# Shahriar1638/Hybrid-Language-Music-Clustering-VAE

Hardware: AMD Instinct MI355X
Metric: clips/sec mel+VAE train step, 128-mel x 128-frame, bs=256, 1/2/4/8 MI355X (higher is better)
Workload: dtype bf16; 1 GPU; Convolutional_VAE audio-only (BASELINE config[1]): PCM[256,65024] -> HIP mel-dB 128x128 -> z-score -> VAE fwd+bwd+Adam; per_gpu_batch=256, global_batch=256, mel=128x128, params=13304961, parallelism=dp1, world_size=1, launch=single process, pcm_batches=5 distinct batches in rotation (333 MB), execution=eager launches

## Files before the change

### hybrid-language-music-clustering-vae_amd/_lib.py

```python
from __future__ import annotations

import ctypes as C
import os

import numpy as np
import torch

_HERE = os.path.dirname(os.path.abspath(__file__))
LIB_PATH = os.environ.get("HLMC_LIB") or os.path.join(_HERE, "libhlmc.so")

c_int, c_i64, c_f32, c_f64, c_vp, c_char_p = C.c_int, C.c_int64, C.c_float, C.c_double, C.c_void_p, C.c_char_p
P_vp = C.POINTER(c_vp)
P_i64 = C.POINTER(c_i64)

HLMC_F32, HLMC_BF16 = 0, 1
NET_HYBRID, NET_CVAE, NET_SIMPLE = 0, 1, 2

_SIGS = {
    "hlmc_version": (c_int, []),
    "hlmc_last_error": (c_char_p, []),
    "hlmc_device_status": (c_int, [c_int]),
    "hlmc_test_bn_fused": (c_int, [c_i64, c_int]),
    "hlmc_mel_plan_create": (c_int, [c_int, c_int, c_int, c_int, c_f64, c_f64, P_vp]),
    "hlmc_mel_plan_destroy": (c_int, [c_vp]),
    "hlmc_mel_filterbank": (c_int, [c_vp, c_vp]),
    "hlmc_mel_frames": (c_i64, [c_vp, c_i64]),
    "hlmc_mel_workspace": (c_i64, [c_vp, c_i64, c_i64]),
    "hlmc_melspectrogram": (c_int, [c_vp, c_vp, c_vp, c_i64, c_i64, c_vp, c_vp]),
    "hlmc_mel_db": (c_int, [c_vp, c_vp, c_vp, c_i64, c_i64, c_i64, c_f32, c_f32, c_vp, c_vp]),
    "hlmc_mel_db_zscore": (c_int, [c_vp, c_vp, c_vp, c_i64, c_i64, c_i64, c_f32, c_f32, c_vp, c_vp, c_int, c_vp,
                                   c_vp]),
    "hlmc_power_to_db": (c_int, [c_vp, c_vp, c_i64, c_i64, c_int, c_f32, c_f32, c_f32, c_vp, c_vp]),
    "hlmc_mfcc": (c_int, [c_vp, c_vp, c_vp, c_i64, c_i64, c_int, c_vp, c_vp]),
    "hlmc_spectral_shape": (c_int, [c_vp, c_vp, c_vp, c_i64, c_i64, c_f64, c_vp]),
    "hlmc_zcr_rms": (c_int, [c_vp, c_vp, c_vp, c_i64, c_i64, c_vp, c_vp]),
    "hlmc_chroma_workspace": (c_i64, [c_vp, c_i64, c_i64]),
    "hlmc_chroma_stft": (c_int, [c_vp, c_vp, c_vp, c_i64, c_i64, c_vp, c_vp, c_vp]),
    "hlmc_row_mean_std": (c_int, [c_vp, c_vp, c_i64, c_i64, c_vp, c_vp]),
    "hlmc_colstats_workspace": (c_i64, [c_i64, c_i64]),
    "hlmc_colstats_sum": (c_int, [c_vp, c_vp, c_i64, c_i64, c_vp, c_vp]),
    "hlmc_colstats_centered": (c_int, [c_vp, c_vp, c_i64, c_i64, c_vp, c_vp, c_vp, c_vp]),
    "hlmc_zscore_apply": (c_int, [c_vp, c_vp, c_i64, c_i64, c_vp, c_vp, c_int, c_vp]),
    "hlmc_net_create": (c_int, [c_int, P_i64, c_int, c_int, P_vp]),
    "hlmc_net_destroy": (c_int, [c_vp]),
    "hlmc_net_num_params": (c_int, [c_vp]),
    "hlmc_net_param_info": (c_int, [c_vp, c_int, c_char_p, c_int, C.POINTER(c_int), P_i64]),
    "hlmc_net_num_bn": (c_int, [c_vp]),
    "hlmc_net_state_bytes": (c_i64, [c_vp]),
    "hlmc_net_workspace_bytes": (c_i64, [c_vp, c_i64]),
    "hlmc_net_bind": (c_int, [c_vp, P_vp, P_vp, P_vp, P_vp, c_vp]),
    "hlmc_net_forward": (c_int, [c_vp, c_vp, c_i64, c_int, c_vp, c_vp, c_vp, c_vp, c_vp, c_vp, c_vp, c_vp, c_vp,
                                 c_vp, c_vp]),
    "hlmc_net_encode": (c_int, [c_vp, c_vp, c_i64, c_int, c_vp, c_vp, c_vp, c_vp, c_vp, c_vp]),
    "hlmc_net_decode": (c_int, [c_vp, c_vp, c_i64, c_int, c_vp, c_vp, c_vp, c_vp, c_vp, c_vp]),
    "hlmc_net_backward": (c_int, [c_vp, c_vp, c_i64, c_vp, c_vp, c_vp, c_vp, c_vp]),
    "hlmc_net_adam_step": (c_int, [c_vp, c_vp, P_vp, P_vp, c_f32, c_f32, c_f32, c_f32, c_f32, c_int]),
    "hlmc_net_set_trust_packs": (c_int, [c_vp, c_int]),
    "hlmc_net_adam_step_dev": (c_int, [c_vp, c_vp, P_vp, P_vp, c_vp]),
    "hlmc_adam_coef": (c_int, [c_f32, c_f32, c_f32, c_f32, c_f32, c_int, c_vp]),
    "hlmc_net_set_overlap_adam": (c_int, [c_vp, c_int]),
    "hlmc_net_set_rng": (c_int, [c_vp, C.c_uint64, C.c_uint64]),
    "hlmc_net_get_rng": (c_int, [c_vp, C.POINTER(C.c_uint64), C.POINTER(C.c_uint64)]),
    "hlmc_randn": (c_int, [c_vp, c_vp, c_i64, C.c_uint64, C.c_uint64]),
    "hlmc_net_settle": (c_int, [c_vp, c_vp]),
    "hlmc_net_grad_buckets": (c_int, [c_vp, C.POINTER(c_int), c_int]),
    "hlmc_net_set_bucket_sync": (c_int, [c_vp, c_int]),
    "hlmc_net_bucket_wait": (c_int, [c_vp, c_int, c_vp]),
    "hlmc_probe_arm": (c_int, [c_int, c_int]),
    "hlmc_probe_read": (c_int, [C.POINTER(c_int), C.POINTER(c_f64), C.POINTER(c_f64), C.POINTER(c_f64),
                                C.POINTER(c_f32), c_int]),
    "hlmc_loss_workspace": (c_i64, [c_i64, c_i64, c_i64]),
    "hlmc_loss_sums": (c_int, [c_vp, c_vp, c_vp, c_i64, c_vp, c_vp, c_i64, c_vp, c_vp, c_i64, c_vp, c_vp]),
    "hlmc_loss_backward": (c_int, [c_vp, c_vp, c_vp, c_i64, c_vp, c_vp, c_vp, c_i64, c_vp, c_vp, c_vp, c_i64,
                                   c_vp, c_vp, c_vp]),
    "hlmc_loss_sums_backward": (c_int, [c_vp, c_vp, c_vp, c_i64, c_vp, c_vp, c_vp, c_i64, c_vp, c_vp, c_vp, c_i64,
                                        c_vp, c_vp, c_vp, c_vp, c_vp]),
    "hlmc_adam_scratch_bytes": (c_i64, [c_int]),
    "hlmc_adam_step": (c_int, [c_vp, c_int, P_vp, P_vp, P_vp, P_vp, P_i64, c_f32, c_f32, c_f32, c_f32, c_f32,
                               c_int, c_vp]),
    "hlmc_km_center": (c_int, [c_vp, c_vp, c_i64, c_int, c_vp, c_vp, c_vp]),
    "hlmc_km_sqdist_rows": (c_int, [c_vp, c_vp, c_i64, c_int, P_i64, c_int, c_vp]),
    "hlmc_km_assign": (c_int, [c_vp, c_vp, c_i64, c_int, c_vp, c_int, c_vp, c_vp, c_vp]),
    "hlmc_km_sums": (c_int, [c_vp, c_vp, c_i64, c_int, c_vp, c_int, c_vp, c_vp]),
    "hlmc_km_sums_workspace": (c_i64, [c_i64, c_int]),
    "hlmc_km_sums_part": (c_int, [c_vp, c_vp, c_i64, c_int, c_vp, c_int, c_vp, c_vp, c_vp, c_i64]),
    "hlmc_km_rowdist": (c_int, [c_vp, c_vp, c_i64, c_int, c_vp, c_vp, c_vp]),
    "hlmc_km_inertia": (c_int, [c_vp, c_vp, c_i64, c_int, c_vp, c_vp, c_vp, c_vp]),
    "hlmc_op_bn_bwd_workspace": (c_i64, [c_int]),
    "hlmc_op_bn_bwd": (c_int, [c_vp, c_int, c_vp, c_vp, c_i64, c_int, c_vp, c_vp, c_vp, c_vp, c_vp, c_vp, c_vp, c_vp, c_vp,
                               c_i64]),
    "hlmc_km_assign_batch": (c_int, [c_vp, c_vp, c_i64, c_int, c_vp, c_int, c_int, C.c_uint64, c_vp, c_vp, c_vp]),
    "hlmc_km_sums_batch": (c_int, [c_vp, c_vp, c_i64, c_int, c_vp, c_int, c_int, C.c_uint64, c_vp, c_vp, c_vp, c_i64]),
    "hlmc_km_update_batch": (c_int, [c_vp, c_int, c_int, c_int, C.c_uint64, c_vp, c_vp, c_vp, c_vp, c_vp]),
    "hlmc_km_pp_search": (c_int, [c_vp, c_i64, c_int, c_int, c_vp, c_int, C.POINTER(C.c_int32), C.POINTER(c_f64), c_vp,
                                  c_vp]),
    "hlmc_km_pp_dist": (c_int, [c_vp, c_vp, c_i64, c_int, c_int, c_int, c_vp, c_vp, c_int, C.POINTER(C.c_int32), c_vp]),
    "hlmc_km_inertia_batch": (c_int, [c_vp, c_vp, c_i64, c_int, c_vp, c_int, c_vp, c_int, c_vp, c_vp]),
    "hlmc_silhouette_workspace": (c_i64, [c_i64, c_int]),
    "hlmc_silhouette": (c_int, [c_vp, c_vp, c_i64, c_int, c_vp, c_int, c_vp, c_vp, c_vp, c_i64]),
    "hlmc_cluster_scores_workspace": (c_i64, [c_int, c_int]),
    "hlmc_cluster_scores": (c_int, [c_vp, c_vp, c_i64, c_int, c_vp, c_int, c_vp, c_vp, c_i64]),
    "hlmc_dbscan_workspace": (c_i64, [c_i64, c_int]),
    "hlmc_dbscan_neighbors": (c_int, [c_vp, c_vp, c_i64, c_int, C.POINTER(c_f64), c_int, c_vp, c_vp, c_vp, c_i64]),
    "hlmc_dbscan_labels": (c_int, [c_vp, c_i64, c_int, c_int, c_int, c_vp, c_vp, c_i64, c_vp, c_vp, c_vp]),
    "hlmc_ward_workspace": (c_i64, [c_i64]),
    "hlmc_ward_pdist": (c_int, [c_vp, c_vp, c_i64, c_int, c_vp]),
    "hlmc_ward_chain": (c_int, [c_vp, c_i64, c_vp, c_vp, c_vp, c_vp, c_vp, c_vp, c_i64]),
    "hlmc_pca_workspace": (c_i64, [c_i64, c_int]),
    "hlmc_pca_cov": (c_int, [c_vp, c_vp, c_i64, c_int, c_vp, c_vp, c_vp, c_i64]),
# ... 97 lines not shown
```

### hybrid-language-music-clustering-vae_amd/csrc/capi.cpp

```cpp
#include <algorithm>
#include <cmath>
#include <cstring>
#include <memory>
#include <vector>

#include "engine.hpp"
#include "features.hpp"

namespace hlmc {

static thread_local std::string g_err;
void set_error(const std::string& msg) { g_err = msg; }
const char* get_error() { return g_err.c_str(); }
static int device_status_ok() {
    const unsigned st = ops::dev_status_take(false);
    if (st == 0) return HLMC_OK;
    set_error("device status " + std::to_string(st) +
              (st & kDevBnCountTimeout ? ": a one-launch BatchNorm backward's grid-wide arrival count timed out (grid not "
                                         "co-resident); that launch's dgamma / dbeta / dy are NaN" : "") +
              " -- clear with hlmc_device_status(1)");
    return HLMC_EDEVICE;
}

namespace probe {
// ... 213 lines not shown
    for (int i = 0; i < n.n_bn; ++i) {
        n.RM.push_back(running[2 * i]);
        n.RV.push_back(running[2 * i + 1]);
    }
    n.NBT.assign(nbt, nbt + n.n_bn);
    for (size_t i = 0; i < np; ++i) HLMC_CHECK_ARG(n.P[i] && n.G[i], "NULL parameter / grad pointer");
    n.state = reinterpret_cast<char*>(state);
    n.packs_valid = false;
    return n.bind_state(nullptr);
}
int hlmc_net_forward(hlmc_net* h, void* stream, int64_t batch, int train, const float* in0, const float* in1,
                     const float* in2, const float* eps, const uint8_t* dropout, float* recon, float* recon_text,
                     float* mu, float* logvar, float* z, void* ws) {
    HLMC_CHECK_ARG(h && ws && batch > 0, "bad arguments");
    HLMC_CHECK_ARG(!h->impl->P.empty(), "net is not bound");
    ForwardArgs a{batch, train, in0, in1, in2, eps, dropout, recon, recon_text, mu, logvar, z, ws, false};
    return h->impl->forward(S(stream), a);
}
int hlmc_net_encode(hlmc_net* h, void* stream, int64_t batch, int train, const float* in0, const float* in1,
                    const float* in2, float* mu, float* logvar, void* ws) {
    HLMC_CHECK_ARG(h && ws && batch > 0, "bad arguments");
    HLMC_CHECK_ARG(!h->impl->P.empty(), "net is not bound");
    ForwardArgs a{batch, train, in0, in1, in2, nullptr, nullptr, nullptr, nullptr, mu, logvar, nullptr, ws, true};
    return h->impl->forward(S(stream), a);
}
int hlmc_net_decode(hlmc_net* h, void* stream, int64_t batch, int train, const float* z, const float* cond,
                    const uint8_t* dropout, float* recon, float* recon_text, void* ws) {
    HLMC_CHECK_ARG(h && ws && batch > 0 && z && recon, "bad arguments");
    HLMC_CHECK_ARG(!h->impl->P.empty(), "net is not bound");
    ForwardArgs a{batch, train, z, nullptr, cond, nullptr, dropout, recon, recon_text, nullptr, nullptr, nullptr, ws,
                  false, true};
    return h->impl->forward(S(stream), a);
}
int hlmc_net_backward(hlmc_net* h, void* stream, int64_t batch, const float* d_recon, const float* d_recon_text,
                      const float* d_mu, const float* d_logvar, void* ws) {
    HLMC_CHECK_ARG(h && ws && d_recon && d_mu && d_logvar, "bad arguments");
    HLMC_TRY(device_status_ok());
    BackwardArgs a{batch, d_recon, d_recon_text, d_mu, d_logvar, ws};
    return h->impl->backward(S(stream), a);
}

int hlmc_net_adam_step(hlmc_net* h, void* stream, float* const* exp_avg, float* const* exp_avg_sq, float lr, float b1,
                       float b2, float eps, float wd, int step) {
    HLMC_CHECK_ARG(h && exp_avg && exp_avg_sq && step >= 1, "bad arguments");
    HLMC_CHECK_ARG(!h->impl->P.empty(), "net is not bound");
    return h->impl->adam_step(S(stream), exp_avg, exp_avg_sq, ops::AdamArgs{lr, b1, b2, eps, wd, step});
}
int hlmc_net_adam_step_dev(hlmc_net* h, void* stream, float* const* exp_avg, float* const* exp_avg_sq,
                           const float* coef_dev) {
    HLMC_CHECK_ARG(h && exp_avg && exp_avg_sq && coef_dev, "bad arguments");
    HLMC_CHECK_ARG(!h->impl->P.empty(), "net is not bound");
    return h->impl->adam_step(S(stream), exp_avg, exp_avg_sq, ops::AdamArgs{0.f, 0.f, 0.f, 0.f, 0.f, 1}, coef_dev);
}
int hlmc_adam_coef(float lr, float b1, float b2, float eps, float wd, int step, float* out6) {
    HLMC_CHECK_ARG(out6 && step >= 1, "bad arguments");
    ops::adam_coef_host(ops::AdamArgs{lr, b1, b2, eps, wd, step}, out6);
    return HLMC_OK;
}
int hlmc_net_set_trust_packs(hlmc_net* h, int trust) {
    HLMC_CHECK_ARG(h, "net is NULL");
    h->impl->trust_packs = trust != 0;
    if (!trust) h->impl->packs_valid = false;
    return HLMC_OK;
}
int hlmc_net_settle(hlmc_net* h, void* stream) {
    HLMC_CHECK_ARG(h, "net is NULL");
    return h->impl->settle(S(stream));
}
int hlmc_net_set_rng(hlmc_net* h, uint64_t seed, uint64_t offset) {
    HLMC_CHECK_ARG(h && offset % 4 == 0, "net is NULL / offset not a multiple of 4");
    h->impl->rng_seed = seed;
    h->impl->rng_offset = offset;
    return HLMC_OK;
}
int hlmc_net_get_rng(const hlmc_net* h, uint64_t* seed, uint64_t* offset) {
    HLMC_CHECK_ARG(h && seed && offset, "NULL argument");
    *seed = h->impl->rng_seed;
    *offset = h->impl->rng_offset;
    return HLMC_OK;
}
int hlmc_randn(void* stream, float* out, int64_t n, uint64_t seed, uint64_t offset) {
    return ops::randn(S(stream), out, n, seed, offset);
}
int hlmc_net_set_overlap_adam(hlmc_net* h, int enable) {
    HLMC_CHECK_ARG(h, "net is NULL");
    h->impl->overlap_adam = enable != 0;
    return HLMC_OK;
}
int hlmc_net_grad_buckets(const hlmc_net* h, int* starts, int cap) {
    HLMC_CHECK_ARG(h && starts && cap > 0, "NULL argument");
    const auto& b = h->impl->bucket_starts;
    for (int k = 0; k < (int)b.size() && k < cap; ++k) starts[k] = b[k];
    return (int)b.size();
}
int hlmc_net_set_bucket_sync(hlmc_net* h, int enable) {
    HLMC_CHECK_ARG(h, "net is NULL");
    h->impl->bucket_sync = enable != 0;
    return HLMC_OK;
}
int hlmc_net_bucket_wait(hlmc_net* h, int k, void* stream) {
    HLMC_CHECK_ARG(h, "net is NULL");
    auto& ev = h->impl->bucket_ev;
    HLMC_CHECK_ARG(h->impl->bucket_sync && k >= 0 && k < (int)ev.size() && ev[k],
                   "bucket events not recorded (hlmc_net_set_bucket_sync + hlmc_net_backward first)");
    HLMC_HIP(hipStreamWaitEvent(S(stream), ev[k], 0));
    return HLMC_OK;
// ... 249 lines not shown
```

### hybrid-language-music-clustering-vae_amd/csrc/engine.cpp

```cpp
#include "engine.hpp"

#include <algorithm>
#include <climits>
#include <cstdlib>
#include <functional>

namespace hlmc {
namespace {

constexpr float kBnEps = 1e-5f;
constexpr float kBnMomentum = 0.1f;
constexpr int ENC_CH[7] = {1, 32, 64, 128, 256, 512, 512};
constexpr int DEC_CH[7] = {512, 512, 256, 128, 64, 32, 1};

inline int pad8(int64_t n) { return (int)((n + 7) & ~int64_t(7)); }

struct WgradQueue {
    using Fn = std::function<int(hipStream_t, Ws)>;
    bool on = true;
    Ws ws_main{nullptr, 0};
    Ws ws_own{nullptr, 0};

    WgradQueue() = default;
    WgradQueue(const WgradQueue&) = delete;
// ... 121 lines not shown
            p.ld1 = q.ld1 = pad8(p.d0);
            p.off0 = A.take((size_t)2 * p.d0 * p.ld0 * sizeof(T));
            q.off0 = p.off0 + (size_t)p.d0 * p.ld0 * sizeof(T);
            p.off1 = A.take((size_t)p.d1 * p.ld1 * sizeof(T));
            q.off1 = A.take((size_t)q.d1 * q.ld1 * sizeof(T));
        }
        for (auto& p : packs) {
            if (!p.taps) continue;
            ++njobs;
            if (p.off0 != SIZE_MAX) continue;
            p.ld0 = p.taps == 1 ? pad8(p.d1) : p.d1;
            p.ld1 = p.taps == 1 ? pad8(p.d0) : p.d0;
            p.off0 = A.take((size_t)p.d0 * p.taps * p.ld0 * sizeof(T));
            p.off1 = A.take((size_t)p.d1 * p.taps * p.ld1 * sizeof(T));
        }
        jobs_off = A.take(sizeof(ops::AdamJob) * std::max<size_t>(1, njobs));
        ajobs_off = A.take(sizeof(ops::AdamJob) * std::max<size_t>(1, params.size()));
        state_size = A.used;
    }
    size_t state_bytes() const override { return state_size; }
    ops::AdamJob job_for(size_t i, float* m, float* v) const {
        const Pack& p = packs[i];
        ops::AdamJob j{P[i], G[i], m, v, nullptr, nullptr, params[i].numel(), 0, 0, 0, 0, 0, 0, 0};
        if (p.taps) {
            j.p0 = state + p.off0;
            j.p1 = state + p.off1;
            j.d0 = p.d0; j.d1 = p.d1; j.taps = p.taps; j.ld0 = p.ld0; j.ld1 = p.ld1;
        }
        return j;
    }
    std::vector<ops::AdamJob> pjobs;
    int bind_state(hipStream_t s) override {
        pjobs.clear();
        pack_tiles = 0;
        for (size_t i = 0; i < packs.size(); ++i) {
            if (!packs[i].taps) continue;
            ops::AdamJob j = job_for(i, nullptr, nullptr);
            j.tile0 = pack_tiles;
            pack_tiles += ops::adam_job_tiles(j);
            pjobs.push_back(j);
        }
        if (!pjobs.empty())
            HLMC_HIP(hipMemcpyAsync(state + jobs_off, pjobs.data(), pjobs.size() * sizeof(ops::AdamJob), hipMemcpyHostToDevice, s));
        ajobs_m.clear();
        HLMC_HIP(hipStreamSynchronize(s));
        return HLMC_OK;
    }
    int pack_all(hipStream_t s) {
        if (trust_packs && packs_valid) return HLMC_OK;
        HLMC_TRY(ops::pack<T>(s, reinterpret_cast<const ops::AdamJob*>(state + jobs_off), njobs, pack_tiles));
        packs_valid = true;
        return HLMC_OK;
    }
    int adam_step(hipStream_t s, float* const* m, float* const* v, const ops::AdamArgs& a, const float* coef_dev) override {
        const size_t np = params.size();
        if (ajobs_m.size() != np || !std::equal(ajobs_m.begin(), ajobs_m.end(), m) ||
            !std::equal(ajobs_v.begin(), ajobs_v.end(), v)) {
            ajobs_m.assign(m, m + np);
            ajobs_v.assign(v, v + np);
            ajobs.clear();
            adam_tiles = 0;
            for (size_t i = 0; i < np; ++i) {
                ops::AdamJob j = job_for(i, m[i], v[i]);
                j.tile0 = adam_tiles;
                adam_tiles += ops::adam_job_tiles(j);
                ajobs.push_back(j);
            }
            HLMC_HIP(hipMemcpyAsync(state + ajobs_off, ajobs.data(), ajobs.size() * sizeof(ops::AdamJob),
                                    hipMemcpyHostToDevice, s));
        }
        const auto* jd = reinterpret_cast<const ops::AdamJob*>(state + ajobs_off);
        if (join_pending) {
            const int tsplit = ajobs[this->late_params].tile0;
            HLMC_TRY(wq.wait_prelate(s));
            HLMC_TRY(ops::adam_pack<T>(s, jd, (int)np, adam_tiles, a, coef_dev, tsplit));
            HLMC_TRY(wq.join(s));
            join_pending = false;
            HLMC_TRY(ops::adam_pack<T>(s, jd, (int)np, tsplit, a, coef_dev, 0));
        } else {
            HLMC_TRY(ops::adam_pack<T>(s, jd, (int)np, adam_tiles, a, coef_dev));
        }
        packs_valid = true;
        return HLMC_OK;
    }
    T* P0(int w) const { return reinterpret_cast<T*>(state + packs[w].off0); }
    T* P1(int w) const { return reinterpret_cast<T*>(state + packs[w].off1); }
    int ld0(int w) const { return packs[w].ld0; }
    int ld1(int w) const { return packs[w].ld1; }

    char* ws = nullptr;
    Ws scratch{nullptr, 0};
    size_t scratch_off = 0, scratch2_off = 0, scratch_bytes = 0;
    int64_t planned_B = -1;
    size_t ws_total = 0;

    T* AT(size_t off) const { return reinterpret_cast<T*>(ws + off); }
    float* AF(size_t off) const { return reinterpret_cast<float*>(ws + off); }
    uint8_t* AU8(size_t off) const { return reinterpret_cast<uint8_t*>(ws + off); }

    void need(size_t b) { scratch_bytes = std::max(scratch_bytes, b); }
    size_t xf_total = 0, xb_total = 0, xf_base = 0, xb_base = 0;
    bool bwd_acc_clean = false;
    int zero_acc_fwd(hipStream_t s) {
        if (xf_total + xb_total) HLMC_HIP(hipMemsetAsync(ws + xf_base, 0, xf_total + xb_total, s));
        bwd_acc_clean = true;
        return HLMC_OK;
    }
    int zero_acc_bwd(hipStream_t s) {
        if (!bwd_acc_clean && xb_total) HLMC_HIP(hipMemsetAsync(ws + xb_base, 0, xb_total, s));
        bwd_acc_clean = false;
        return HLMC_OK;
    }

    virtual void plan(Arena& A, int64_t B) = 0;
    size_t ws_bytes(int64_t B) override {
        if (B != planned_B) {
            Arena A;
            scratch_bytes = 0;
            xf_total = xb_total = 0;
            plan(A, B);
            scratch_off = A.take(scratch_bytes + 256);
            scratch2_off = A.take(scratch_bytes + 256);
            xf_base = A.take(xf_total);
            xb_base = A.take(xb_total);
            ws_total = A.used;
            planned_B = B;
        }
        return ws_total;
    }
    void set_ws(void* w) {
        ws = reinterpret_cast<char*>(w);
        scratch = Ws{reinterpret_cast<float*>(ws + scratch_off), scratch_bytes + 256};
        wq.ws_main = scratch;
        wq.ws_own = Ws{reinterpret_cast<float*>(ws + scratch2_off), scratch_bytes + 256};
    }

    WgradQueue wq;
    bool join_pending = false;
    ~NetT() override {
        for (auto e : this->bucket_ev) (void)hipEventDestroy(e);
    }
    static constexpr int side_batch() { return 2; }
    static constexpr int dense_batch() { return 2; }
    bool tail_overlap() const { return wq.on && this->overlap_adam && !this->bucket_sync && this->late_params > 0; }
    int prelate(hipStream_t s) { return tail_overlap() ? wq.record_prelate(s) : (int)HLMC_OK; }
    int settle(hipStream_t s) override {
        if (!join_pending) return HLMC_OK;
        join_pending = false;
        return wq.join(s);
    }
    int finish_backward(hipStream_t s) {
        if (tail_overlap()) {
            join_pending = true;
            return HLMC_OK;
        }
        return wq.join(s);
    }
    int mark(hipStream_t s, int k) {
        if (!this->bucket_sync) return HLMC_OK;
        HLMC_CHECK_ARG(k >= 0 && k < (int)this->bucket_ev.size(), "bucket index");
        if (wq.on && k + 1 < (int)this->bucket_ev.size()) return wq.record_bucket(s, this->bucket_ev[k]);
        HLMC_HIP(hipEventRecord(this->bucket_ev[k], s));
        return HLMC_OK;
    }

    int begin_forward(hipStream_t s, const ForwardArgs& a) {
        HLMC_CHECK_ARG(a.B >= 2 || !a.train, "BatchNorm in train mode needs batch >= 2");
        ws_bytes((int)a.B);
        set_ws(a.ws);
        HLMC_TRY(settle(s));
        HLMC_TRY(pack_all(s));
        if (a.train) HLMC_TRY(zero_acc_fwd(s));
        this->last_full_forward = !a.encode_only && !a.decode_only;
        return HLMC_OK;
    }
    int begin_backward(hipStream_t s, const BackwardArgs& a) {
        HLMC_CHECK_ARG((int)a.B == planned_B, "backward batch differs from the last forward");
        HLMC_CHECK_ARG(this->last_full_forward, "backward needs a full hlmc_net_forward (not encode / decode)");
        set_ws(a.ws);
        HLMC_TRY(wq.init());
        if (this->bucket_sync && this->bucket_ev.size() != this->bucket_starts.size()) {
            for (auto e : this->bucket_ev) (void)hipEventDestroy(e);
            this->bucket_ev.assign(this->bucket_starts.size(), nullptr);
            for (auto& e : this->bucket_ev) HLMC_HIP(hipEventCreateWithFlags(&e, hipEventDisableTiming));
        }
        HLMC_TRY(settle(s));
        return zero_acc_bwd(s);
    }

    int reparam(hipStream_t s, const float* eps_in, const float* mu, const float* lv, float* eps_keep, int B, int L,
                T* z, int ldz, float* mu_out, float* lv_out) {
        if (eps_in) return ops::reparam_fwd<T>(s, mu, lv, eps_in, B, L, z, ldz, mu_out, lv_out, eps_keep);
        return ops::reparam_rng<T>(s, mu, lv, this->rng_seed, take_rng(B, L), B, L, eps_keep, z, ldz, mu_out, lv_out);
    }
    uint64_t take_rng(int B, int L) {
        const uint64_t off = this->rng_offset;
        this->rng_offset += ((uint64_t)B * L + 3) & ~uint64_t(3);
        return off;
    }
    int latent_out(hipStream_t s, const ForwardArgs& a, const float* mu, const float* lv, int64_t nl) {
        const ops::CopySeg cs[2] = {{a.mu, mu, nl}, {a.logvar, lv, nl}};
        return ops::copy_segments(s, cs, 2);
    }
    int heads_fwd(hipStream_t s, const ForwardArgs& a, const T* x, int ldx, int B, int L, int mu_w, int mu_b, int lv_b,
                  float* mu, float* lv, float* eps_keep, T* z, int ldz) {
        const int K = (int)params[mu_w].shape[1];
        int S = 0;
        HLMC_TRY(ops::linear_partials<T>(s, x, ldx, B, K, P0(mu_w), ld0(mu_w), 2 * L, scratch, &S));
        if (a.encode_only)
            return ops::heads_reparam<T>(s, scratch.p, S, B, L, P[mu_b], P[lv_b], mu, lv, a.mu, a.logvar, nullptr, 0, 0,
                                         nullptr, nullptr, 0);
// ... 934 lines not shown
```

### hybrid-language-music-clustering-vae_amd/csrc/engine.hpp

```cpp
#pragma once
#include <memory>
#include <string>
#include <vector>

#include "ops.hpp"

namespace hlmc {

struct ParamInfo {
    std::string name;
    std::vector<int64_t> shape;
    int64_t numel() const {
        int64_t n = 1;
        for (auto d : shape) n *= d;
        return n;
    }
};

struct Arena {
    size_t used = 0;
    size_t take(size_t bytes) {
        size_t o = used;
        used += (bytes + 255) & ~size_t(255);
        return o;
// ... 1 lines not shown
};

struct ForwardArgs {
    int64_t B;
    int train;
    const float* in0;
    const float* in1;
    const float* in2;
    const float* eps;
    const uint8_t* dropout;
    float* recon;
    float* recon_text;
    float* mu;
    float* logvar;
    float* z;
    void* ws;
    bool encode_only;
    bool decode_only = false;
};

struct BackwardArgs {
    int64_t B;
    const float* d_recon;
    const float* d_recon_text;
    const float* d_mu;
    const float* d_logvar;
    void* ws;
};

class NetBase {
  public:
    virtual ~NetBase() = default;
    int kind = 0, dtype = 0;
    std::vector<ParamInfo> params;
    int n_bn = 0;

    std::vector<float*> P, G, RM, RV;
    std::vector<int64_t*> NBT;
    char* state = nullptr;

    int add_param(const std::string& name, std::vector<int64_t> shape) {
        params.push_back({name, std::move(shape)});
        return (int)params.size() - 1;
    }
    int add_bn() { return n_bn++; }

    virtual size_t state_bytes() const = 0;
    virtual size_t ws_bytes(int64_t B) = 0;
    virtual int bind_state(hipStream_t s) = 0;
    virtual int forward(hipStream_t s, const ForwardArgs& a) = 0;
    virtual int backward(hipStream_t s, const BackwardArgs& a) = 0;
    virtual int adam_step(hipStream_t s, float* const* m, float* const* v, const ops::AdamArgs& a,
                          const float* coef_dev = nullptr) = 0;
    bool trust_packs = false;
    bool packs_valid = false;

    std::vector<int> bucket_starts{0};
    std::vector<hipEvent_t> bucket_ev;
    bool bucket_sync = false;

    int late_params = 0;
    bool overlap_adam = false;
    bool last_full_forward = false;
    uint64_t rng_seed = 0, rng_offset = 0;
    virtual int settle(hipStream_t s) = 0;
};

int make_net(int kind, const int64_t* cfg, int ncfg, int dtype, std::unique_ptr<NetBase>* out);

}
```

### hybrid-language-music-clustering-vae_amd/train.py

```python
from __future__ import annotations

import os

import torch

from . import _lib as L
from .models import ConditionalVAE, HybridVAE, VAE


class Trainer:
    def __init__(self, model, lr=1e-4, betas=(0.9, 0.999), eps=1e-8, weight_decay=0.0, beta=None, text_weight=None,
                 process_group=None, distributed=False, grad_dtype=torch.float32, broadcast_buffers=True):
        self.model = model
        self.distributed = distributed or process_group is not None
        self.process_group = process_group
        self.broadcast_buffers = bool(broadcast_buffers) and self.distributed
        self.bn_flat = model._flatten_bn_buffers() if self.broadcast_buffers else None
        self.kind = "simple" if isinstance(model, VAE) else ("cvae" if isinstance(model, ConditionalVAE) else "hybrid")
        self.net = model._native_net()
        dev = next(model.parameters()).device
        self.device = dev
        self.params = list(model.parameters())
        self.gflat = model._gflat
        self.grads = model._grad_views
        n = self.gflat.numel()
        self.m = torch.zeros(n, dtype=torch.float32, device=dev)
        self.v = torch.zeros(n, dtype=torch.float32, device=dev)
        mv, vv, off = [], [], 0
        for p in self.params:
            mv.append(self.m[off:off + p.numel()])
            vv.append(self.v[off:off + p.numel()])
            off += p.numel()
        self.lr, self.betas, self.eps, self.wd = lr, betas, eps, weight_decay
        self.step_count = 0
        if beta is None:
            beta = {"hybrid": 1.0, "cvae": 4.0, "simple": 0.8}[self.kind]
        if text_weight is None:
            text_weight = {"hybrid": 350.0, "cvae": 200.0, "simple": 0.0}[self.kind]
        self.beta, self.text_weight = float(beta), float(text_weight)
        self.grad_dtype = grad_dtype
        self.buckets = self._bucket_ranges()
        self._comm = None
        self._fwd_done = None
        self._rng_key = 0
        if self.distributed:
            import torch.distributed as dist
            rank = dist.get_rank(process_group) if process_group is not None else dist.get_rank()
            self._rng_key = rank_rng_key(rank)
            if rank:
                seed, off = model.get_rng_state()
                model.set_rng_state((keyed_seed(seed, self._rng_key), off))
        if self.distributed and dev.type == "cuda":
            self._fwd_done = torch.cuda.Event()
            L.check(L.lib().hlmc_net_set_bucket_sync(self.net.h, 1), "hlmc_net_set_bucket_sync")
            self._comm = torch.cuda.Stream(device=dev)
        else:
            on = int(os.environ.get("HLMC_OVERLAP_ADAM", "0") == "1")
            L.check(L.lib().hlmc_net_set_overlap_adam(self.net.h, on), "hlmc_net_set_overlap_adam")
        self._mv = (L.vp_array([t.data_ptr() for t in mv]), L.vp_array([t.data_ptr() for t in vv]))
        self._graph = False
        self._coef_dev = torch.zeros(6, dtype=torch.float32, device=dev)
        self._coef_ring = torch.zeros(1024, 6, dtype=torch.float32).pin_memory() if dev.type == "cuda" else None
        L.check(L.lib().hlmc_net_set_trust_packs(self.net.h, 1))
        self._cache = {}

    def _buffers(self, B):
        if B not in self._cache:
            dev = self.device
            m = self.model
            out = m._alloc_outputs(B, dev)
            d = {k: torch.empty_like(v) for k, v in out.items()}
            ws = self.net.new_workspace(B, dev)
            na = out["recon"].numel()
            nt = out["recon_text"].numel() if "recon_text" in out else 0
            nl = out["mu"].numel()
            lws = torch.empty(max(16, int(L.lib().hlmc_loss_workspace(na, nt, nl))), dtype=torch.uint8, device=dev)
            sums = torch.zeros(3, dtype=torch.float64, device=dev)
            if self.kind == "simple":
                coef = torch.tensor([2.0 / na, 0.0, self.beta / nl], device=dev)
            else:
                coef = torch.tensor([2.0, 2.0 * self.text_weight, self.beta], device=dev)
            self._cache[B] = dict(out=out, d=d, ws=ws, lws=lws, sums=sums, coef=coef, n=(na, nt, nl))
        return self._cache[B]

    def state_dict(self):
        seed, off = self.model.get_rng_state()
        return {"step": self.step_count, "exp_avg": self.m.detach().clone(), "exp_avg_sq": self.v.detach().clone(),
                "rng": (keyed_seed(seed, -self._rng_key), off)}

    def load_state_dict(self, sd):
        self.step_count = int(sd["step"])
        self.m.copy_(sd["exp_avg"])
        self.v.copy_(sd["exp_avg_sq"])
        seed, off = sd["rng"]
        self.model.set_rng_state((keyed_seed(int(seed), self._rng_key), int(off)))

    def step(self, in0, in1=None, in2=None, eps=None, dropout=None, before_adam=None):
        lib = L.lib()
        s = L.stream()
        B = in0.shape[0]
        if self.broadcast_buffers:
            self._check_bn_flat()
        c = self._buffers(B)
        out, d = c["out"], c["d"]
        if eps is None and self._graph:
            eps = torch.randn(B, self.model.latent_dim, device=self.device)
        if self.kind == "simple" and dropout is None:
            dropout = self.model.make_dropout_mask(B, self.device)
        L.check(lib.hlmc_net_forward(self.net.h, s, B, 1, L.ptr(in0), L.ptr(in1), L.ptr(in2), L.ptr(eps),
                                     L.ptr(dropout), L.ptr(out["recon"]), L.ptr(out.get("recon_text")),
                                     L.ptr(out["mu"]), L.ptr(out["logvar"]), L.ptr(out.get("z")), c["ws"].data_ptr()),
                "hlmc_net_forward")
        bcast = None
        if self.broadcast_buffers:
            bcast = self._broadcast_buffers_after_forward()
        na, nt, nl = c["n"]
        rt, t = out.get("recon_text"), (in1 if nt else None)
        L.check(lib.hlmc_loss_sums_backward(s, L.ptr(out["recon"]), L.ptr(in0), na, L.ptr(d["recon"]), L.ptr(rt),
                                            L.ptr(t), nt, L.ptr(d.get("recon_text")), L.ptr(out["mu"]),
                                            L.ptr(out["logvar"]), nl, c["coef"].data_ptr(), L.ptr(d["mu"]),
                                            L.ptr(d["logvar"]), c["sums"].data_ptr(), c["lws"].data_ptr()),
                "hlmc_loss_sums_backward")
        L.check(lib.hlmc_net_backward(self.net.h, s, B, L.ptr(d["recon"]), L.ptr(d.get("recon_text")), L.ptr(d["mu"]),
                                      L.ptr(d["logvar"]), c["ws"].data_ptr()), "hlmc_net_backward")
        if self.distributed:
            if self._comm is not None:
                self._allreduce_overlapped(bcast)
            else:
                self.allreduce_grads()
        if before_adam is not None:
            L.check(lib.hlmc_net_settle(self.net.h, s), "hlmc_net_settle")
            before_adam()
        if self._graph:
            L.check(lib.hlmc_net_adam_step_dev(self.net.h, s, *self._mv, self._coef_dev.data_ptr()),
                    "hlmc_net_adam_step_dev")
            return c["sums"]
        self.step_count += 1
        b1, b2 = self.betas
        L.check(lib.hlmc_net_adam_step(self.net.h, s, *self._mv, float(self.lr), float(b1), float(b2), float(self.eps),
                                       float(self.wd), self.step_count), "hlmc_net_adam_step")
        return c["sums"]

    def prepare_step_coefficients(self):
        self.step_count += 1
        slot = self._coef_ring[self.step_count % self._coef_ring.shape[0]]
        b1, b2 = self.betas
        L.check(L.lib().hlmc_adam_coef(float(self.lr), float(b1), float(b2), float(self.eps), float(self.wd),
                                       self.step_count, slot.data_ptr()), "hlmc_adam_coef")
        self._coef_dev.copy_(slot, non_blocking=True)

    def release(self):
        L.check(L.lib().hlmc_net_set_trust_packs(self.net.h, 0))
        L.check(L.lib().hlmc_net_set_overlap_adam(self.net.h, 0))

    def _bucket_ranges(self):
        offs = [0]
        for p in self.params:
            offs.append(offs[-1] + p.numel())
        cap = 64
        starts = (L.c_int * cap)()
        nb = L.lib().hlmc_net_grad_buckets(self.net.h, starts, cap)
        if nb < 0:
            L.check(nb, "hlmc_net_grad_buckets")
        return bucket_ranges(list(starts)[:nb], offs)

    def _check_bn_flat(self):
        bns = [m for m in self.model.modules() if isinstance(m, torch.nn.modules.batchnorm._BatchNorm)]
        if bns and bns[0].running_mean.data_ptr() != self.bn_flat.data_ptr():
            raise L.HLMCError("BatchNorm running statistics were replaced after the Trainer was built "
                              "(module._apply / load_state_dict(assign=True)); build a new Trainer")

    def _broadcast_buffers_after_forward(self):
        import torch.distributed as dist
        src = dist.get_global_rank(self.process_group, 0) if self.process_group is not None else 0
        if self._comm is None:
# ... 119 lines not shown
```

### include/hlmc.h

```cpp
#ifndef HLMC_H_
#define HLMC_H_

#include <stdint.h>

#ifdef __cplusplus
extern "C" {
#endif

enum hlmc_status {
    HLMC_OK = 0,
    HLMC_EINVAL = -1,
    HLMC_EHIP = -2,
    HLMC_EUNSUP = -3,
    HLMC_EDEVICE = -4,
};

enum hlmc_dtype { HLMC_F32 = 0, HLMC_BF16 = 1 };

int hlmc_version(void);
const char* hlmc_last_error(void);
int hlmc_device_status(int clear);
int hlmc_test_bn_fused(int64_t max_elems, int spin_max);

typedef struct hlmc_mel_plan hlmc_mel_plan;
// ... 8 lines not shown
int hlmc_mel_db(const hlmc_mel_plan* plan, void* stream, const float* pcm, int64_t batch, int64_t n_samples,
                int64_t t_keep, float amin, float top_db, float* out, void* ws);
int hlmc_mel_db_zscore(const hlmc_mel_plan* plan, void* stream, const float* pcm, int64_t batch, int64_t n_samples,
                       int64_t t_keep, float amin, float top_db, const double* mean, const double* scale,
                       int out_dtype, void* out, void* ws);
int hlmc_power_to_db(void* stream, const float* S, int64_t batch, int64_t per_clip, int ref_max, float ref_value,
                     float amin, float top_db, float* out, void* ws);
int hlmc_mfcc(const hlmc_mel_plan* plan, void* stream, const float* pcm, int64_t batch, int64_t n_samples,
              int n_mfcc, float* out, void* ws);
int hlmc_spectral_shape(const hlmc_mel_plan* plan, void* stream, const float* pcm, int64_t batch, int64_t n_samples,
                        double roll_percent, double* out);
int hlmc_zcr_rms(const hlmc_mel_plan* plan, void* stream, const float* pcm, int64_t batch, int64_t n_samples,
                 double* zcr, float* rms);
int64_t hlmc_chroma_workspace(const hlmc_mel_plan* plan, int64_t batch, int64_t n_samples);
int hlmc_chroma_stft(const hlmc_mel_plan* plan, void* stream, const float* pcm, int64_t batch, int64_t n_samples,
                     float* out, double* tuning, void* ws);
int hlmc_row_mean_std(void* stream, const float* x, int64_t rows, int64_t cols, float* mean, float* std);
int64_t hlmc_colstats_workspace(int64_t n, int64_t cols);
int hlmc_colstats_sum(void* stream, const float* x, int64_t n, int64_t cols, double* sum, void* ws);
int hlmc_colstats_centered(void* stream, const float* x, int64_t n, int64_t cols, const double* mean, double* corr,
                           double* m2, void* ws);
int hlmc_zscore_apply(void* stream, const float* x, int64_t n, int64_t cols, const double* mean, const double* scale,
                      int out_dtype, void* out);

typedef struct hlmc_net hlmc_net;
enum hlmc_net_kind { HLMC_NET_HYBRID = 0, HLMC_NET_CVAE = 1, HLMC_NET_SIMPLE = 2 };

int hlmc_net_create(int kind, const int64_t* cfg, int ncfg, int dtype, hlmc_net** out);
int hlmc_net_destroy(hlmc_net* net);
int hlmc_net_num_params(const hlmc_net* net);
int hlmc_net_param_info(const hlmc_net* net, int i, char* name, int cap, int* ndim, int64_t* shape);
int hlmc_net_num_bn(const hlmc_net* net);
int64_t hlmc_net_state_bytes(const hlmc_net* net);
int64_t hlmc_net_workspace_bytes(const hlmc_net* net, int64_t batch);
int hlmc_net_bind(hlmc_net* net, float* const* params, float* const* grads, float* const* running,
                  int64_t* const* nbt, void* state);
int hlmc_net_forward(hlmc_net* net, void* stream, int64_t batch, int train, const float* in0, const float* in1,
                     const float* in2, const float* eps, const uint8_t* dropout, float* recon, float* recon_text,
                     float* mu, float* logvar, float* z, void* ws);
int hlmc_net_set_rng(hlmc_net* net, uint64_t seed, uint64_t offset);
int hlmc_net_get_rng(const hlmc_net* net, uint64_t* seed, uint64_t* offset);
int hlmc_randn(void* stream, float* out, int64_t n, uint64_t seed, uint64_t offset);
int hlmc_net_encode(hlmc_net* net, void* stream, int64_t batch, int train, const float* in0, const float* in1,
                    const float* in2, float* mu, float* logvar, void* ws);
int hlmc_net_decode(hlmc_net* net, void* stream, int64_t batch, int train, const float* z, const float* cond,
                    const uint8_t* dropout, float* recon, float* recon_text, void* ws);
int hlmc_net_backward(hlmc_net* net, void* stream, int64_t batch, const float* d_recon, const float* d_recon_text,
                      const float* d_mu, const float* d_logvar, void* ws);

int hlmc_net_adam_step(hlmc_net* net, void* stream, float* const* exp_avg, float* const* exp_avg_sq, float lr,
                       float beta1, float beta2, float eps, float weight_decay, int step);
int hlmc_net_adam_step_dev(hlmc_net* net, void* stream, float* const* exp_avg, float* const* exp_avg_sq,
                           const float* coef_dev);
int hlmc_adam_coef(float lr, float beta1, float beta2, float eps, float weight_decay, int step, float* out6);
int hlmc_net_set_trust_packs(hlmc_net* net, int trust);

int hlmc_net_set_overlap_adam(hlmc_net* net, int enable);
int hlmc_net_settle(hlmc_net* net, void* stream);

int hlmc_net_grad_buckets(const hlmc_net* net, int* starts, int cap);
int hlmc_net_set_bucket_sync(hlmc_net* net, int enable);
int hlmc_net_bucket_wait(hlmc_net* net, int k, void* stream);

int hlmc_probe_arm(int mask, int max_launches);
int hlmc_probe_read(int* launches, double* total_ms, double* flops, double* bytes, float* ms_each, int cap_each);

int hlmc_loss_sums(void* stream, const float* ra, const float* a, int64_t na, const float* rt, const float* t,
                   int64_t nt, const float* mu, const float* lv, int64_t nl, double* sums3, void* ws);
int64_t hlmc_loss_workspace(int64_t na, int64_t nt, int64_t nl);
int hlmc_loss_backward(void* stream, const float* ra, const float* a, int64_t na, float* dra, const float* rt,
                       const float* t, int64_t nt, float* drt, const float* mu, const float* lv, int64_t nl,
                       const float* coef, float* dmu, float* dlv);
int hlmc_loss_sums_backward(void* stream, const float* ra, const float* a, int64_t na, float* dra, const float* rt,
                            const float* t, int64_t nt, float* drt, const float* mu, const float* lv, int64_t nl,
                            const float* coef, float* dmu, float* dlv, double* sums3, void* ws);

int hlmc_adam_step(void* stream, int n, float* const* params, const float* const* grads, float* const* exp_avg,
                   float* const* exp_avg_sq, const int64_t* numel, float lr, float beta1, float beta2, float eps,
                   float weight_decay, int step, void* scratch);
int64_t hlmc_adam_scratch_bytes(int n);

int hlmc_km_center(void* stream, const float* X, int64_t n, int d, float* mean, float* var, float* Xc);
int hlmc_km_sqdist_rows(void* stream, const float* X, int64_t n, int d, const int64_t* cand, int ncand, float* out);
int hlmc_km_assign(void* stream, const float* X, int64_t n, int d, const float* centers, int k, int32_t* labels,
                   const int32_t* labels_old, int32_t* n_changed);
int hlmc_km_sums(void* stream, const float* X, int64_t n, int d, const int32_t* labels, int k, float* sums,
                 float* weight);
int64_t hlmc_km_sums_workspace(int64_t n, int k);
int hlmc_km_sums_part(void* stream, const float* X, int64_t n, int d, const int32_t* labels, int k, float* sums,
                      float* weight, void* ws, int64_t ws_bytes);
int hlmc_km_rowdist(void* stream, const float* X, int64_t n, int d, const float* centers, const int32_t* labels,
                    float* out);
int hlmc_km_inertia(void* stream, const float* X, int64_t n, int d, const float* centers, const int32_t* labels,
                    float* out, float* tmp);

int hlmc_km_assign_batch(void* stream, const float* X, int64_t n, int d, const float* centers, int k, int R,
                         uint64_t active, int32_t* labels, const int32_t* labels_old, int32_t* n_changed);
int hlmc_km_sums_batch(void* stream, const float* X, int64_t n, int d, const int32_t* labels, int k, int R,
                       uint64_t active, float* sums, float* weight, void* ws, int64_t ws_bytes);
int hlmc_km_update_batch(void* stream, int k, int d, int R, uint64_t active, const float* sums, const float* weight,
                         const float* C_old, float* C_new, float* info);
int hlmc_km_pp_search(void* stream, int64_t n, int R, int T, const float* prev, int prevT, const int32_t* best,
                      const double* rvals, int64_t* cand, int32_t* amb);
int hlmc_km_pp_dist(void* stream, const float* X, int64_t n, int d, int R, int T, const int64_t* cand, const float* prev,
                    int prevT, const int32_t* best, float* out);
int hlmc_km_inertia_batch(void* stream, const float* X, int64_t n, int d, const float* centers, int k,
// ... 58 lines not shown
```

Baseline: 144,200 clips/s.

## Overlap Adam updates for finished gradient buckets with remaining backward pass

Adds a fused backward+Adam entry point that launches Adam on the wgrad side queue for the first gradient buckets as soon as the backward pass marks them complete. The remaining parameters are updated after backward ends. The aim is to hide optimizer time behind the tail of the backward pass on single-GPU runs. In exchange it adds cross-queue ordering complexity and extra launches, and it is disabled under distributed, graph or overlap modes.

```diff
diff --git a/hybrid-language-music-clustering-vae_amd/_lib.py b/hybrid-language-music-clustering-vae_amd/_lib.py
--- a/hybrid-language-music-clustering-vae_amd/_lib.py
+++ b/hybrid-language-music-clustering-vae_amd/_lib.py
@@ -55,6 +55,9 @@
     "hlmc_net_decode": (c_int, [c_vp, c_vp, c_i64, c_int, c_vp, c_vp, c_vp, c_vp, c_vp, c_vp]),
     "hlmc_net_backward": (c_int, [c_vp, c_vp, c_i64, c_vp, c_vp, c_vp, c_vp, c_vp]),
     "hlmc_net_adam_step": (c_int, [c_vp, c_vp, P_vp, P_vp, c_f32, c_f32, c_f32, c_f32, c_f32, c_int]),
+    "hlmc_net_backward_adam": (c_int, [c_vp, c_vp, c_i64, c_vp, c_vp, c_vp, c_vp, c_vp, P_vp, P_vp, c_f32, c_f32, c_f32,
+                                       c_f32, c_f32, c_int]),
+    "hlmc_net_adam_launches": (c_int, [c_vp]),
     "hlmc_net_set_trust_packs": (c_int, [c_vp, c_int]),
     "hlmc_net_adam_step_dev": (c_int, [c_vp, c_vp, P_vp, P_vp, c_vp]),
     "hlmc_adam_coef": (c_int, [c_f32, c_f32, c_f32, c_f32, c_f32, c_int, c_vp]),
diff --git a/hybrid-language-music-clustering-vae_amd/csrc/capi.cpp b/hybrid-language-music-clustering-vae_amd/csrc/capi.cpp
--- a/hybrid-language-music-clustering-vae_amd/csrc/capi.cpp
+++ b/hybrid-language-music-clustering-vae_amd/csrc/capi.cpp
@@ -289,6 +289,16 @@
     HLMC_CHECK_ARG(!h->impl->P.empty(), "net is not bound");
     return h->impl->adam_step(S(stream), exp_avg, exp_avg_sq, ops::AdamArgs{0.f, 0.f, 0.f, 0.f, 0.f, 1}, coef_dev);
 }
+int hlmc_net_backward_adam(hlmc_net* h, void* stream, int64_t batch, const float* d_recon, const float* d_recon_text,
+                           const float* d_mu, const float* d_logvar, void* ws, float* const* exp_avg,
+                           float* const* exp_avg_sq, float lr, float b1, float b2, float eps, float wd, int step) {
+    HLMC_CHECK_ARG(h && ws && d_recon && d_mu && d_logvar && exp_avg && exp_avg_sq && step >= 1, "bad arguments");
+    HLMC_CHECK_ARG(!h->impl->P.empty(), "net is not bound");
+    HLMC_TRY(device_status_ok());
+    BackwardArgs a{batch, d_recon, d_recon_text, d_mu, d_logvar, ws};
+    return h->impl->backward_adam(S(stream), a, exp_avg, exp_avg_sq, ops::AdamArgs{lr, b1, b2, eps, wd, step});
+}
+int hlmc_net_adam_launches(const hlmc_net* h) { return h ? h->impl->adam_launches : -1; }
 int hlmc_adam_coef(float lr, float b1, float b2, float eps, float wd, int step, float* out6) {
     HLMC_CHECK_ARG(out6 && step >= 1, "bad arguments");
     ops::adam_coef_host(ops::AdamArgs{lr, b1, b2, eps, wd, step}, out6);
diff --git a/hybrid-language-music-clustering-vae_amd/csrc/engine.cpp b/hybrid-language-music-clustering-vae_amd/csrc/engine.cpp
--- a/hybrid-language-music-clustering-vae_amd/csrc/engine.cpp
+++ b/hybrid-language-music-clustering-vae_amd/csrc/engine.cpp
@@ -197,7 +197,7 @@
         packs_valid = true;
         return HLMC_OK;
     }
-    int adam_step(hipStream_t s, float* const* m, float* const* v, const ops::AdamArgs& a, const float* coef_dev) override {
+    int adam_jobs(hipStream_t s, float* const* m, float* const* v) {
         const size_t np = params.size();
         if (ajobs_m.size() != np || !std::equal(ajobs_m.begin(), ajobs_m.end(), m) ||
             !std::equal(ajobs_v.begin(), ajobs_v.end(), v)) {
@@ -214,18 +214,62 @@
             HLMC_HIP(hipMemcpyAsync(state + ajobs_off, ajobs.data(), ajobs.size() * sizeof(ops::AdamJob),
                                     hipMemcpyHostToDevice, s));
         }
-        const auto* jd = reinterpret_cast<const ops::AdamJob*>(state + ajobs_off);
+        return HLMC_OK;
+    }
+    const ops::AdamJob* adam_jobs_dev() const { return reinterpret_cast<const ops::AdamJob*>(state + ajobs_off); }
+    int adam_step(hipStream_t s, float* const* m, float* const* v, const ops::AdamArgs& a, const float* coef_dev) override {
+        HLMC_TRY(adam_jobs(s, m, v));
+        this->adam_launches = 0;
+        return adam_rest(s, a, coef_dev, adam_tiles);
+    }
+    int adam_rest(hipStream_t s, const ops::AdamArgs& a, const float* coef_dev, int end) {
+        const int np = (int)params.size();
+        const auto* jd = adam_jobs_dev();
         if (join_pending) {
             const int tsplit = ajobs[this->late_params].tile0;
             HLMC_TRY(wq.wait_prelate(s));
-            HLMC_TRY(ops::adam_pack<T>(s, jd, (int)np, adam_tiles, a, coef_dev, tsplit));
+            HLMC_TRY(ops::adam_pack<T>(s, jd, np, end, a, coef_dev, tsplit));
             HLMC_TRY(wq.join(s));
             join_pending = false;
-            HLMC_TRY(ops::adam_pack<T>(s, jd, (int)np, tsplit, a, coef_dev, 0));
+            HLMC_TRY(ops::adam_pack<T>(s, jd, np, tsplit, a, coef_dev, 0));
+            this->adam_launches += 2;
         } else {
-            HLMC_TRY(ops::adam_pack<T>(s, jd, (int)np, adam_tiles, a, coef_dev));
+            HLMC_TRY(ops::adam_pack<T>(s, jd, np, end, a, coef_dev));
+            this->adam_launches += 1;
         }
         packs_valid = true;
+        return HLMC_OK;
+    }
+
+    static int adam_buckets_env() {
+        static const int n = [] {
+            const char* e = std::getenv("HLMC_ADAM_BUCKETS");
+            return e && e[0] ? std::max(0, std::atoi(e)) : 2;
+        }();
+        return n;
+    }
+    int early_n = 0, early_from = 0;
+    ops::AdamArgs early_args{};
+    int backward_adam(hipStream_t s, const BackwardArgs& b, float* const* m, float* const* v,
+                      const ops::AdamArgs& a) override {
+        HLMC_TRY(adam_jobs(s, m, v));
+        this->adam_launches = 0;
+        early_from = adam_tiles;
+        early_args = a;
+        early_n = (this->bucket_sync || this->overlap_adam)
+                      ? 0 : std::min(adam_buckets_env(), (int)this->bucket_starts.size() - 1);
+        const int rc = backward(s, b);
+        early_n = 0;
+        if (rc != HLMC_OK) return rc;
+        return adam_rest(s, a, nullptr, early_from);
+    }
+    int early_adam(hipStream_t s, int k) {
+        const int np = (int)params.size(), begin = ajobs[this->bucket_starts[k]].tile0, end = early_from;
+        const auto* jd = adam_jobs_dev();
+        const ops::AdamArgs a = early_args;
+        HLMC_TRY(wq.run(s, [=](hipStream_t q, Ws) { return ops::adam_pack<T>(q, jd, np, end, a, nullptr, begin); }));
+        early_from = begin;
+        this->adam_launches += 1;
         return HLMC_OK;
     }
     T* P0(int w) const { return reinterpret_cast<T*>(state + packs[w].off0); }
@@ -302,6 +346,7 @@
         return wq.join(s);
     }
     int mark(hipStream_t s, int k) {
+        if (k < early_n) return early_adam(s, k);
         if (!this->bucket_sync) return HLMC_OK;
         HLMC_CHECK_ARG(k >= 0 && k < (int)this->bucket_ev.size(), "bucket index");
         if (wq.on && k + 1 < (int)this->bucket_ev.size()) return wq.record_bucket(s, this->bucket_ev[k]);
diff --git a/hybrid-language-music-clustering-vae_amd/csrc/engine.hpp b/hybrid-language-music-clustering-vae_amd/csrc/engine.hpp
--- a/hybrid-language-music-clustering-vae_amd/csrc/engine.hpp
+++ b/hybrid-language-music-clustering-vae_amd/csrc/engine.hpp
@@ -77,6 +77,9 @@
     virtual int backward(hipStream_t s, const BackwardArgs& a) = 0;
     virtual int adam_step(hipStream_t s, float* const* m, float* const* v, const ops::AdamArgs& a,
                           const float* coef_dev = nullptr) = 0;
+    virtual int backward_adam(hipStream_t s, const BackwardArgs& b, float* const* m, float* const* v,
+                              const ops::AdamArgs& a) = 0;
+    int adam_launches = 0;
     bool trust_packs = false;
     bool packs_valid = false;
 
diff --git a/hybrid-language-music-clustering-vae_amd/train.py b/hybrid-language-music-clustering-vae_amd/train.py
--- a/hybrid-language-music-clustering-vae_amd/train.py
+++ b/hybrid-language-music-clustering-vae_amd/train.py
@@ -57,6 +57,7 @@
         else:
             on = int(os.environ.get("HLMC_OVERLAP_ADAM", "0") == "1")
             L.check(L.lib().hlmc_net_set_overlap_adam(self.net.h, on), "hlmc_net_set_overlap_adam")
+        self._fused_adam = not self.distributed and os.environ.get("HLMC_OVERLAP_ADAM", "0") != "1"
         self._mv = (L.vp_array([t.data_ptr() for t in mv]), L.vp_array([t.data_ptr() for t in vv]))
         self._graph = False
         self._coef_dev = torch.zeros(6, dtype=torch.float32, device=dev)
@@ -121,6 +122,14 @@
                                             L.ptr(out["logvar"]), nl, c["coef"].data_ptr(), L.ptr(d["mu"]),
                                             L.ptr(d["logvar"]), c["sums"].data_ptr(), c["lws"].data_ptr()),
                 "hlmc_loss_sums_backward")
+        if self._fused_adam and before_adam is None and not self._graph:
+            self.step_count += 1
+            b1, b2 = self.betas
+            L.check(lib.hlmc_net_backward_adam(self.net.h, s, B, L.ptr(d["recon"]), L.ptr(d.get("recon_text")),
+                                               L.ptr(d["mu"]), L.ptr(d["logvar"]), c["ws"].data_ptr(), *self._mv,
+                                               float(self.lr), float(b1), float(b2), float(self.eps), float(self.wd),
+                                               self.step_count), "hlmc_net_backward_adam")
+            return c["sums"]
         L.check(lib.hlmc_net_backward(self.net.h, s, B, L.ptr(d["recon"]), L.ptr(d.get("recon_text")), L.ptr(d["mu"]),
                                       L.ptr(d["logvar"]), c["ws"].data_ptr()), "hlmc_net_backward")
         if self.distributed:
diff --git a/include/hlmc.h b/include/hlmc.h
--- a/include/hlmc.h
+++ b/include/hlmc.h
@@ -84,6 +84,11 @@
                        float beta1, float beta2, float eps, float weight_decay, int step);
 int hlmc_net_adam_step_dev(hlmc_net* net, void* stream, float* const* exp_avg, float* const* exp_avg_sq,
                            const float* coef_dev);
+int hlmc_net_backward_adam(hlmc_net* net, void* stream, int64_t batch, const float* d_recon,
+                           const float* d_recon_text, const float* d_mu, const float* d_logvar, void* ws,
+                           float* const* exp_avg, float* const* exp_avg_sq, float lr, float beta1, float beta2,
+                           float eps, float weight_decay, int step);
+int hlmc_net_adam_launches(const hlmc_net* net);
 int hlmc_adam_coef(float lr, float beta1, float beta2, float eps, float weight_decay, int step, float* out6);
 int hlmc_net_set_trust_packs(hlmc_net* net, int trust);
 
```

New measurement: 145,100 clips/s (median of 2 runs). About the same (+0.7%).
